# DIAGNijmegen/prostateMR_3D-CAD-csPCa

Measured on AMD Instinct MI355X. Metric: train-step volumes/sec (whole job), M1 (20,160,160,3), higher is better.
Workload: dtype bf16; 1 GPU; C3 M1 full hierarchical-probabilistic dense_skip+deep_supervision latents (3,2,1,0) (20,160,160,3); batch_per_gpu=2, global_batch=2, params=67254246, parallelism=dp1, hip_graph=True

## Files before the change

### prostatemr_3d-cad-cspca_amd/csrc/conv_mfma.h

```cpp
#pragma once
#include "common.h"
#include "gather.h"
#include "cdna4.h"

#define MF_MAX_TAPS 27
#define MF_MAX_CLASSES 8

struct MfmaP {
    const void* src[M1_MAX_SRC];
    int srcC[M1_MAX_SRC];
    int srcSeg[M1_MAX_SRC];
    int nsrc, CC, spt;
    int ID, IH, IW;
    void* out;
    int OC, OCn;
    int nout;
    void* outs[M1_MAX_SRC]; int outC[M1_MAX_SRC]; int outOff[M1_MAX_SRC + 1]; int outAcc[M1_MAX_SRC];
    int OD, OH, OW, N;
    const void* wp;
    const float* bias;
    const float* bias2; int bias_split;
    int mode, sd, sh, sw, pd, ph, pw;
    int nclasses;
    int cls_ntaps[MF_MAX_CLASSES], cls_first[MF_MAX_CLASSES], cls_kpad[MF_MAX_CLASSES];
    long long cls_woff[MF_MAX_CLASSES];
    signed char tdd[MF_MAX_TAPS], tdh[MF_MAX_TAPS], tdw[MF_MAX_TAPS];
    int tap_pk[MF_MAX_TAPS];
    int accumulate;
    int ksplit;
    float* acc32;
    long long slab_elems;
    int aligned;
    int korder;
    const void* ib_x;
    const float* ib_stats; const float* ib_gamma; const float* ib_beta; float ib_slope;
    int tps;
    float* stat_partial;
    int stat_tiles;
};

struct OutRef { void* base; int C, col, acc; };
__device__ __forceinline__ OutRef m1_out_ref(const MfmaP& p, int oc) {
    if (p.nout == 0) return OutRef{p.out, p.OC, oc, p.accumulate};
    int m = 0;
    while (m + 1 < p.nout && oc >= p.outOff[m + 1]) ++m;
    return OutRef{p.outs[m], p.outC[m], oc - p.outOff[m], p.outAcc[m]};
}

__device__ __forceinline__ float m1_bias_at(const MfmaP& p, int oc) {
    if (p.bias_split > 0 && oc >= p.bias_split) return p.bias2 ? p.bias2[oc - p.bias_split] : 0.f;
    return p.bias ? p.bias[oc] : 0.f;
}

template <typename T> struct MT;
template <> struct MT<bf16_t> { static constexpr int SEG = 8; };
template <> struct MT<float> { static constexpr int SEG = 4; };


bool m1_halo_conv_supported(const MfmaP& mp, int OCpad);
int m1_halo_conv_stat_parts(const MfmaP& mp, int OCpad);
int m1_halo_conv(const MfmaP& mp, int OCpad, hipStream_t st);

bool m1_pw_conv_supported(const MfmaP& mp, int OCpad, int BN);
int m1_pw_conv_stat_parts(const MfmaP& mp, int OCpad, int BN);
int m1_pw_conv(const MfmaP& mp, int OCpad, int BN, hipStream_t st);
```

### prostatemr_3d-cad-cspca_amd/csrc/conv_mfma.hip

```cpp
#include "common.h"
#include "gather.h"
#include "reduce.h"

#include "conv_mfma.h"
#include "conv_t3.h"
#include <stdlib.h>

template <typename T>
__device__ __forceinline__ uint4 load_partial_seg(const T* p, int n) {
    constexpr int SEG = MT<T>::SEG;
    union { uint4 v; T e[SEG]; } u;
    u.v = make_uint4(0, 0, 0, 0);
#pragma unroll
    for (int k = 0; k < SEG; ++k) if (k < n) u.e[k] = p[k];
    return u.v;
}

__device__ __forceinline__ unsigned lds_addr_of(const void* p) { return (unsigned)(unsigned long long)(lptr_t)p; }

template <typename T, int BM, int BN, int WM, int WN, int KC, bool GLDS, int KG = 1>
__global__ void __launch_bounds__(WM * WN * 64 * KG) conv_mfma_kernel(MfmaP p) {
#if defined(__HIP_DEVICE_COMPILE__)
    constexpr int NTHR = WM * WN * 64, NW = WM * WN;
    static_assert(KG == 1 || GLDS, "K groups: LDS-DMA path only");
    constexpr int SEG = MT<T>::SEG;
    constexpr int TM = BM / WM / 16, TN = BN / WN / 16;
    constexpr int A_BYTES = BM * 64, B_BYTES = BN * 64;
    constexpr int A_LD = BM * 4 / NTHR;
    constexpr int B_LD = (BN * 4 + NTHR - 1) / NTHR;
    static_assert((NW == 4 || NW == 8 || NW == 16) && (BM * 4) % NTHR == 0 && BN % 16 == 0, "tile config");

    extern __shared__ __attribute__((aligned(16))) unsigned char smem[];
    int4* rowinfo = reinterpret_cast<int4*>(smem);
    int* outrow = reinterpret_cast<int*>(rowinfo + BM);
    const T** s_src = reinterpret_cast<const T**>(outrow + BM);
    int* s_srcC = reinterpret_cast<int*>(s_src + M1_MAX_SRC);
    int* s_srcSeg = s_srcC + M1_MAX_SRC;
    int* s_tap = s_srcSeg + M1_MAX_SRC;
    int* s_tdl = s_tap + MF_MAX_TAPS;
    constexpr int TBL_BYTES = (BM * 20 + M1_MAX_SRC * 16 + 2 * MF_MAX_TAPS * 4 + 15) / 16 * 16;
    const int kg = KG > 1 ? __builtin_amdgcn_readfirstlane((int)threadIdx.x / NTHR) : 0;
    const int tid = KG > 1 ? (int)threadIdx.x - kg * NTHR : (int)threadIdx.x, lane = tid & 63, wave = tid >> 6;
    constexpr int GROUP_BYTES = 2 * KC * (A_BYTES + B_BYTES);
    unsigned char* A_s = smem + TBL_BYTES + kg * GROUP_BYTES;
    unsigned char* B_s = A_s + 2 * KC * A_BYTES;

    const int wm = wave / WN, wn = wave % WN;
    const int cls = blockIdx.y / p.ksplit, ksp = (blockIdx.y % p.ksplit) * KG + kg;
    const int oc0 = blockIdx.z * BN;

    int pdc = 0, phc = 0, pwc = 0, QD = p.OD, QH = p.OH, QW = p.OW;
    if (p.mode == 1) {
        pwc = cls % p.sw; phc = (cls / p.sw) % p.sh; pdc = cls / (p.sw * p.sh);
        QD = p.OD > pdc ? (p.OD - pdc + p.sd - 1) / p.sd : 0;
        QH = p.OH > phc ? (p.OH - phc + p.sh - 1) / p.sh : 0;
        QW = p.OW > pwc ? (p.OW - pwc + p.sw - 1) / p.sw : 0;
    }
    const long long QV = (long long)QD * QH * QW, Mtot = QV * p.N;
    const long long tile = (long long)(blockIdx.x & 7) * (gridDim.x >> 3) + (blockIdx.x >> 3);
    long long m0 = tile * BM, m_end = Mtot;
    if (p.tps > 0) {
        if (tile >= (long long)p.tps * p.N) return;
        const long long tn = tile / p.tps;
        m0 = tn * QV + (tile - tn * p.tps) * BM; m_end = (tn + 1) * QV;
    }
    if (m0 >= Mtot) return;

    for (int r = tid; r < BM; r += NTHR) {
        const long long m = m0 + r;
        int4 ri = make_int4(-1, 0, 0, 0); int orow = -1;
        if (m < m_end) {
            int n, qw, qh, qd;
            if (Mtot < (1ll << 31)) {
                const unsigned mm = (unsigned)m, qv = (unsigned)QV;
                n = (int)(mm / qv); const unsigned lin = mm - (unsigned)n * qv;
                const unsigned t1 = lin / (unsigned)QW; qw = (int)(lin - t1 * (unsigned)QW);
                qd = (int)(t1 / (unsigned)QH); qh = (int)(t1 - (unsigned)qd * (unsigned)QH);
            } else {
                n = (int)(m / QV); long long lin = m % QV;
                qw = (int)(lin % QW); lin /= QW; qh = (int)(lin % QH); qd = (int)(lin / QH);
            }
            if (p.mode == 0) {
                ri = make_int4(n, qd * p.sd - p.pd, qh * p.sh - p.ph, qw * p.sw - p.pw);
                orow = (int)m;
            } else {
                ri = make_int4(n, qd, qh, qw);
                orow = (int)((((long long)n * p.OD + qd * p.sd + pdc) * p.OH + qh * p.sh + phc) * p.OW + qw * p.sw + pwc);
            }
        }
        rowinfo[r] = ri; outrow[r] = orow;
    }
    if (tid < M1_MAX_SRC) { s_src[tid] = (const T*)p.src[tid]; s_srcC[tid] = p.srcC[tid]; s_srcSeg[tid] = p.srcSeg[tid]; }
    const int ntaps = p.cls_ntaps[cls], tfirst = p.cls_first[cls];
    if (tid < ntaps) {
        const int t = tfirst + tid;
        s_tap[tid] = ((int)p.tdd[t] & 0xff) | (((int)p.tdh[t] & 0xff) << 8) | (((int)p.tdw[t] & 0xff) << 16);
        s_tdl[tid] = ((int)p.tdd[t] * p.IH + (int)p.tdh[t]) * p.IW + (int)p.tdw[t];
    }
    __syncthreads();

    const int spt = p.spt;
    const int nseg = ntaps * spt;
    const int nchunks_all = (nseg + 3) >> 2;
    const int cps = (nchunks_all + p.ksplit * KG - 1) / (p.ksplit * KG);
    const int c_beg = ksp * cps;
    const int nchunks = (c_beg + cps <= nchunks_all ? cps : nchunks_all - c_beg);
    const int kpad = p.cls_kpad[cls];
    const T* wp = (const T*)p.wp + p.cls_woff[cls];

    f32x4_t acc[TM][TN];
#pragma unroll
    for (int i = 0; i < TM; ++i)
#pragma unroll
        for (int j = 0; j < TN; ++j) acc[i][j] = (f32x4_t){0.f, 0.f, 0.f, 0.f};

    uint4 ra[GLDS ? 1 : KC][GLDS ? 1 : A_LD], rb[GLDS ? 1 : KC][GLDS ? 1 : B_LD];
    const int lrow = tid >> 2;
    const int lseg = GLDS ? ((tid & 3) ^ ((-(tid >> 4)) & 3)) : (tid & 3);
    const int wave_u = __builtin_amdgcn_readfirstlane(wave);

    int st_tap = 0, st_s = 0, st_c = 0;
    const T* st_ptr[A_LD];
    auto st_set_tap = [&]() {
        const int tp = s_tap[st_tap];
        const int dd = (signed char)(tp & 0xff), dh = (signed char)((tp >> 8) & 0xff), dw = (signed char)((tp >> 16) & 0xff);
#pragma unroll
        for (int i = 0; i < A_LD; ++i) {
            const int4 ri = rowinfo[lrow + (NTHR / 4) * i];
            const int id = ri.y + dd, ih = ri.z + dh, iw = ri.w + dw;
            st_ptr[i] = nullptr;
            if (ri.x >= 0 && id >= 0 && id < p.ID && ih >= 0 && ih < p.IH && iw >= 0 && iw < p.IW) {
                const long long vox = (((long long)ri.x * p.ID + id) * p.IH + ih) * p.IW + iw;
                st_ptr[i] = s_src[st_s] + vox * s_srcC[st_s] + lseg * SEG;
            }
        }
    };
    constexpr unsigned OOB = 0x80000000u;
    unsigned b_vo[B_LD];
    unsigned rmask[A_LD]; int rvox[A_LD], rbyte[A_LD];
    int tap_db = 0;
    __amdgpu_buffer_rsrc_t rs_a = __builtin_amdgcn_make_buffer_rsrc((void*)p.src[0], 0, 0, 0x00020000);
    auto glds_set_member = [&]() {
        const int sC = __builtin_amdgcn_readfirstlane(s_srcC[st_s]);
#pragma unroll
        for (int i = 0; i < A_LD; ++i) rbyte[i] = (rvox[i] * sC + lseg * SEG) * (int)sizeof(T);
        rs_a = __builtin_amdgcn_make_buffer_rsrc((void*)p.src[__builtin_amdgcn_readfirstlane(st_s)], 0, 0x7fffffff, 0x00020000);
    };
    auto glds_set_tap = [&]() {
        tap_db = __builtin_amdgcn_readfirstlane(s_tdl[st_tap]) * __builtin_amdgcn_readfirstlane(s_srcC[st_s]) * (int)sizeof(T);
    };
    if constexpr (GLDS) {
        int4 ris[A_LD];
#pragma unroll
        for (int i = 0; i < A_LD; ++i) { ris[i] = rowinfo[lrow + (NTHR / 4) * i]; rmask[i] = 0; }
#pragma unroll 9
        for (int t = 0; t < ntaps; ++t) {
            const int tp = s_tap[t];
            const int dd = (signed char)(tp & 0xff), dh = (signed char)((tp >> 8) & 0xff), dw = (signed char)((tp >> 16) & 0xff);
#pragma unroll
            for (int i = 0; i < A_LD; ++i) {
                const bool ok = ris[i].x >= 0 && (unsigned)(ris[i].y + dd) < (unsigned)p.ID && (unsigned)(ris[i].z + dh) < (unsigned)p.IH &&
                                (unsigned)(ris[i].w + dw) < (unsigned)p.IW;
                rmask[i] |= (ok ? 1u : 0u) << t;
            }
        }
#pragma unroll
        for (int i = 0; i < A_LD; ++i) rvox[i] = ((ris[i].x * p.ID + ris[i].y) * p.IH + ris[i].z) * p.IW + ris[i].w;
    }
    if constexpr (GLDS) {
#pragma unroll
        for (int i = 0; i < B_LD; ++i) {
            const int e = tid + NTHR * i;
            b_vo[i] = (unsigned)(((oc0 + (e >> 2)) * kpad + lseg * SEG) * (int)sizeof(T));
        }
    }
    if (p.aligned && nchunks > 0) {
        const int cpt = spt >> 2;
        int c;
        if (p.korder == 2) { const int cg = c_beg / (2 * ntaps), rem = c_beg - cg * 2 * ntaps; st_tap = rem >> 1; c = (cg * 2 + (rem & 1)) * 4 * SEG; }
        else if (p.korder) { const int cg = c_beg / ntaps; st_tap = c_beg - cg * ntaps; c = cg * 4 * SEG; }
        else { st_tap = c_beg / cpt; c = (c_beg - st_tap * cpt) * 4 * SEG; }
        while (c >= s_srcC[st_s]) { c -= s_srcC[st_s]; ++st_s; }
        st_c = c;
        if constexpr (GLDS) { glds_set_member(); glds_set_tap(); } else st_set_tap();
    }

    auto prefetch_stage = [&](int sg) {
#pragma unroll
        for (int kc = 0; kc < KC; ++kc) {
            const int rel = sg * KC + kc;
            const int chunk = c_beg + rel;
            const bool live = rel < nchunks;
#pragma unroll
            for (int i = 0; i < B_LD; ++i) {
                const int e = tid + NTHR * i;
                uint4 v = make_uint4(0, 0, 0, 0);
                if (live && e < BN * 4)
                    v = *reinterpret_cast<const uint4*>(wp + (long long)(oc0 + (e >> 2)) * kpad + (long long)(chunk * 4 + (e & 3)) * SEG);
                rb[kc][i] = v;
            }
            if (!live) {
#pragma unroll
                for (int i = 0; i < A_LD; ++i) ra[kc][i] = make_uint4(0, 0, 0, 0);
            } else if (p.aligned) {
#pragma unroll
                for (int i = 0; i < A_LD; ++i)
                    ra[kc][i] = st_ptr[i] ? *reinterpret_cast<const uint4*>(st_ptr[i] + st_c) : make_uint4(0, 0, 0, 0);
                st_c += 4 * SEG;
                if (st_c >= s_srcC[st_s]) {
                    st_c = 0;
                    if (++st_s == p.nsrc) { st_s = 0; ++st_tap; }
                    if (st_tap < ntaps) st_set_tap();
                }
            } else {
                const int kseg = chunk * 4 + lseg;
                const T* sp = nullptr; int sC = 0, coff = 0, dd = 0, dh = 0, dw = 0;
                const bool kvalid = kseg < nseg;
                if (kvalid) {
                    const int tap_i = kseg / spt;
                    int cs = kseg - tap_i * spt, s = 0;
                    while (cs >= s_srcSeg[s]) { cs -= s_srcSeg[s]; ++s; }
                    sp = s_src[s]; sC = s_srcC[s]; coff = cs * SEG;
                    const int tp = s_tap[tap_i];
                    dd = (signed char)(tp & 0xff); dh = (signed char)((tp >> 8) & 0xff); dw = (signed char)((tp >> 16) & 0xff);
                }
#pragma unroll
                for (int i = 0; i < A_LD; ++i) {
                    const int4 ri = rowinfo[lrow + (NTHR / 4) * i];
                    uint4 v = make_uint4(0, 0, 0, 0);
                    const int id = ri.y + dd, ih = ri.z + dh, iw = ri.w + dw;
                    if (kvalid && coff < sC && ri.x >= 0 && id >= 0 && id < p.ID && ih >= 0 && ih < p.IH && iw >= 0 && iw < p.IW) {
                        const long long vox = (((long long)ri.x * p.ID + id) * p.IH + ih) * p.IW + iw;
                        if (sC % SEG == 0) v = *reinterpret_cast<const uint4*>(sp + vox * sC + coff);
                        else v = load_partial_seg<T>(sp + vox * sC + coff, sC - coff < SEG ? sC - coff : SEG);
                    }
                    ra[kc][i] = v;
                }
            }
        }
    };
    const __amdgpu_buffer_rsrc_t rs_b = __builtin_amdgcn_make_buffer_rsrc((void*)wp, 0, 0x7fffffff, 0x00020000);
    const __amdgpu_buffer_rsrc_t rs_0 = __builtin_amdgcn_make_buffer_rsrc((void*)wp, 0, 0, 0x00020000);
    auto issue_chunk = [&](int kc, int buf, int chunk, const __amdgpu_buffer_rsrc_t ra, const __amdgpu_buffer_rsrc_t rb) {
#pragma unroll
        for (int i = 0; i < B_LD; ++i)
            if ((NW * (i + 1)) * 64 <= BN * 4 || (wave_u + NW * i) * 64 < BN * 4)
                __builtin_amdgcn_raw_ptr_buffer_load_lds(rb, (lptr_t)(B_s + (buf * KC + kc) * B_BYTES + (wave_u + NW * i) * 1024), 16,
                                                         b_vo[i], chunk * 64, 0, 0);
#pragma unroll
        for (int i = 0; i < A_LD; ++i) {
            const unsigned vo = ((rmask[i] >> st_tap) & 1u) ? (unsigned)(rbyte[i] + tap_db) : OOB;
            __builtin_amdgcn_raw_ptr_buffer_load_lds(ra, (lptr_t)(A_s + (buf * KC + kc) * A_BYTES + (wave_u + NW * i) * 1024), 16,
                                                     vo, st_c * (int)sizeof(T), 0, 0);
        }
    };
    auto advance_chunk = [&]() {
        if (p.korder == 2) {
            if (((st_c / (4 * SEG)) & 1) == 0) st_c += 4 * SEG;
            else {
                st_c -= 4 * SEG;
                if (++st_tap == ntaps) {
                    st_tap = 0; st_c += 8 * SEG;
                    if (st_c >= s_srcC[st_s]) { st_c = 0; if (++st_s < p.nsrc) glds_set_member(); }
                }
                if (st_s < p.nsrc) glds_set_tap();
            }
        } else if (p.korder) {
            if (++st_tap == ntaps) {
                st_tap = 0; st_c += 4 * SEG;
                if (st_c >= s_srcC[st_s]) { st_c = 0; if (++st_s < p.nsrc) glds_set_member(); }
            }
            if (st_s < p.nsrc) glds_set_tap();
        } else {
            st_c += 4 * SEG;
            if (st_c >= s_srcC[st_s]) {
                st_c = 0;
                if (++st_s == p.nsrc) { st_s = 0; ++st_tap; }
                if (st_tap < ntaps) { glds_set_member(); glds_set_tap(); }
            }
        }
    };
    auto issue = [&](int sg, int buf) {
        const int rel0 = sg * KC;
        if (rel0 + KC <= nchunks) {
#pragma unroll
            for (int kc = 0; kc < KC; ++kc) { issue_chunk(kc, buf, c_beg + rel0 + kc, rs_a, rs_b); advance_chunk(); }
        } else {
#pragma unroll
            for (int kc = 0; kc < KC; ++kc) {
                const bool live = rel0 + kc < nchunks;
                issue_chunk(kc, buf, c_beg + rel0 + kc, live ? rs_a : rs_0, live ? rs_b : rs_0);
                if (live) advance_chunk();
            }
        }
    };
    auto stage = [&](int buf) {
#pragma unroll
        for (int kc = 0; kc < KC; ++kc) {
#pragma unroll
            for (int i = 0; i < A_LD; ++i) {
                const int row = lrow + (NTHR / 4) * i;
                *reinterpret_cast<uint4*>(A_s + (buf * KC + kc) * A_BYTES + row * 64 + m1_swz64(row, lseg) * 16) = ra[kc][i];
            }
#pragma unroll
            for (int i = 0; i < B_LD; ++i) {
                const int e = tid + NTHR * i;
                if (e < BN * 4) {
                    const int row = e >> 2;
                    *reinterpret_cast<uint4*>(B_s + (buf * KC + kc) * B_BYTES + row * 64 + m1_swz64(row, e & 3) * 16) = rb[kc][i];
                }
            }
        }
    };

    const int fr = lane & 15, fs = lane >> 4;
    const unsigned a_rd = lds_addr_of(A_s) + (wm * (BM / WM) + fr) * 64 + m1_swz64(fr, fs) * 16;
    const unsigned b_rd = lds_addr_of(B_s) + (wn * (BN / WN) + fr) * 64 + m1_swz64(fr, fs) * 16;
    const int nstages = KG > 1 ? (cps + KC - 1) / KC : (nchunks + KC - 1) / KC;
    if (nstages > 0) {
        if constexpr (GLDS) issue(0, 0);
        else { prefetch_stage(0); stage(0); }
    }
    __syncthreads();
    for (int it = 0; it < nstages; ++it) {
        const int buf = it & 1;
        if (it + 1 < nstages) { if constexpr (GLDS) issue(it + 1, buf ^ 1); else prefetch_stage(it + 1); }
        if constexpr (GLDS) {
            u32x4_t af[KC][TM], bfr[KC][TN];
            auto rd = [&](int kc) {
#pragma unroll
                for (int i = 0; i < TM; ++i) af[kc][i] = m1_lds_read128(a_rd + (buf * KC + kc) * A_BYTES + i * 1024);
#pragma unroll
                for (int j = 0; j < TN; ++j) bfr[kc][j] = m1_lds_read128(b_rd + (buf * KC + kc) * B_BYTES + j * 1024);
            };
            rd(0);
#pragma unroll
            for (int kc = 0; kc < KC; ++kc) {
                m1_lds_wait(af[kc][0]);
#pragma unroll
                for (int i = 1; i < TM; ++i) m1_lds_tie(af[kc][i]);
#pragma unroll
                for (int j = 0; j < TN; ++j) m1_lds_tie(bfr[kc][j]);
                if (kc + 1 < KC) rd(kc + 1);
                __builtin_amdgcn_sched_barrier(0);
#pragma unroll
                for (int i = 0; i < TM; ++i)
#pragma unroll
                    for (int j = 0; j < TN; ++j) {
                        if constexpr (sizeof(T) == 2) {
                            acc[i][j] = __builtin_amdgcn_mfma_f32_16x16x32_bf16(__builtin_bit_cast(bf16x8_t, af[kc][i]),
                                                                                __builtin_bit_cast(bf16x8_t, bfr[kc][j]), acc[i][j], 0, 0, 0);
                        } else {
#pragma unroll
                            for (int q = 0; q < 4; ++q)
                                acc[i][j] = __builtin_amdgcn_mfma_f32_16x16x4f32(__uint_as_float(af[kc][i][q]), __uint_as_float(bfr[kc][j][q]), acc[i][j], 0, 0, 0);
                        }
                    }
                if (kc + 1 < KC) __builtin_amdgcn_sched_barrier(0);
            }
        } else {
// ... 85 lines not shown
        constexpr int EPI_BYTES = (int)((BM * CP * sizeof(T) + 15) / 16 * 16), PIPE_BYTES = 2 * KC * (A_BYTES + B_BYTES) * KG;
        float* red = reinterpret_cast<float*>(A_s + (PIPE_BYTES > EPI_BYTES ? PIPE_BYTES : EPI_BYTES));
        constexpr int G = NTHR / BN;
        const int col = tid % BN, rg = tid / BN;
        float s = 0.f, ss = 0.f;
        if (p.ib_x) {
            const int oc = oc0 + col < p.OCn ? oc0 + col : 0, n = (int)(m0 / QV);
            const float mean = p.ib_stats[((long long)n * p.OC + oc) * 2], rstd = p.ib_stats[((long long)n * p.OC + oc) * 2 + 1];
            const float gm = p.ib_gamma[oc], bt = p.ib_beta[oc];
            const T* xb = (const T*)p.ib_x + oc;
            constexpr int RPT = (BM + G - 1) / G;
            if constexpr (RPT > 32) {
                for (int row = rg; row < BM; row += G) {
                    const int orow = outrow[row];
                    if (orow >= 0) {
                        const float xh = (Act<T>::ld(xb + (long long)orow * p.OC) - mean) * rstd;
                        const float dy = Act<T>::ld(C_s + row * CP + col) * lrelu_g(gm * xh + bt, p.ib_slope);
                        s += dy; ss += dy * xh;
                    }
                }
            } else {
            float xv[RPT];
#pragma unroll
            for (int i = 0; i < RPT; ++i) {
                const int row = rg + i * G;
                const int orow = row < BM ? outrow[row] : -1;
                xv[i] = orow >= 0 ? Act<T>::ld(xb + (long long)orow * p.OC) : 0.f;
            }
#pragma unroll
            for (int i = 0; i < RPT; ++i) {
                const int row = rg + i * G;
                if (row < BM && outrow[row] >= 0) {
                    const float xh = (xv[i] - mean) * rstd;
                    const float dy = Act<T>::ld(C_s + row * CP + col) * lrelu_g(gm * xh + bt, p.ib_slope);
                    s += dy; ss += dy * xh;
                }
            }
            }
        } else
        for (int row = rg; row < BM; row += G) {
            if (outrow[row] >= 0) { const float v = Act<T>::ld(C_s + row * CP + col); s += v; ss += v * v; }
        }
        red[tid * 2] = s; red[tid * 2 + 1] = ss;
        __syncthreads();
        if (rg == 0 && oc0 + col < p.OCn) {
            for (int q = 1; q < G; ++q) { s += red[(q * BN + col) * 2]; ss += red[(q * BN + col) * 2 + 1]; }
            float* dst = p.stat_partial + ((tile * p.OC) + oc0 + col) * 2;
            dst[0] = s; dst[1] = ss;
        }
    }
    constexpr int SPR = BN / SEG;
    for (int e = tid; e < BM * SPR; e += NTHR) {
        const int row = e / SPR, cs = e % SPR;
        const int orow = outrow[row];
        const int oc = oc0 + cs * SEG;
        if (orow < 0 || oc >= p.OCn) continue;
        const OutRef o = m1_out_ref(p, oc);
        if (!o.base) continue;
        uint4 v = *reinterpret_cast<const uint4*>(C_s + row * CP + cs * SEG);
        T* dst = (T*)o.base + (long long)orow * o.C + o.col;
        if (o.C % SEG != 0 || (p.nout == 0 && oc + SEG > p.OCn)) {
            union { uint4 q; T e[SEG]; } ve; ve.q = v;
#pragma unroll
            for (int k = 0; k < SEG; ++k) {
                if (oc + k < p.OCn) {
                    float a = Act<T>::ld(&ve.e[k]);
                    if (o.acc) a += Act<T>::ld(dst + k);
                    Act<T>::st(dst + k, a);
                }
            }
            continue;
        }
        if (o.acc) {
            float a[SEG], b[SEG];
            VecIO<T, SEG>::ld(reinterpret_cast<const T*>(&v), a);
            VecIO<T, SEG>::ld(dst, b);
#pragma unroll
            for (int k = 0; k < SEG; ++k) a[k] += b[k];
            VecIO<T, SEG>::st(dst, a);
        } else {
            *reinterpret_cast<uint4*>(dst) = v;
        }
    }
#endif
}

template <typename T, int BM, int BN, int KC, int NTHR, int KG = 1>
static constexpr size_t mfma_smem_bytes() {
    size_t tbl = (BM * 20 + M1_MAX_SRC * 16 + 2 * MF_MAX_TAPS * 4 + 15) / 16 * 16;
    size_t pipe = (size_t)KC * (2 * BM * 64 + 2 * BN * 64) * KG;
    size_t epi = ((size_t)BM * (BN + MT<T>::SEG) * sizeof(T) + 15) / 16 * 16;
    return tbl + (pipe > epi ? pipe : epi) + NTHR * 2 * sizeof(float);
}

struct PackP {
    const float* w; long long wST, wSC, wSO; int oc_off, cc_off, OCn, OCpad, CC;
    const float* w2; long long w2ST, w2SC, w2SO; int oc_split, c_split;
    int nsrc, spt, SEG; int srcC[M1_MAX_SRC], srcSeg[M1_MAX_SRC];
    int nclasses; int cls_ntaps[MF_MAX_CLASSES], cls_first[MF_MAX_CLASSES], cls_kpad[MF_MAX_CLASSES];
    long long cls_woff[MF_MAX_CLASSES];
    unsigned char wtap[MF_MAX_TAPS];
    int korder;
};
__device__ __forceinline__ bool pack_seg_pos(const PackP& p, int cls, int kseg, int* nvalid, int* wtap, int* chan) {
    int tap_i, seg;
    if (p.korder == 2) {
        const int chunk = kseg >> 2, nt = p.cls_ntaps[cls], cg = chunk / (2 * nt), rem = chunk - cg * 2 * nt;
        tap_i = rem >> 1; seg = (cg * 2 + (rem & 1)) * 4 + (kseg & 3);
    } else if (p.korder) {
        const int chunk = kseg >> 2, nt = p.cls_ntaps[cls], cg = chunk / nt;
        tap_i = chunk - cg * nt; seg = cg * 4 + (kseg & 3);
    } else { tap_i = kseg / p.spt; seg = kseg - tap_i * p.spt; }
    int c = 0, s = 0;
    while (s < p.nsrc && seg >= p.srcSeg[s]) { seg -= p.srcSeg[s]; c += p.srcC[s]; ++s; }
    if (s >= p.nsrc || tap_i >= p.cls_ntaps[cls]) { *nvalid = 0; return false; }
    const int rem = p.srcC[s] - seg * p.SEG;
    *nvalid = rem < p.SEG ? rem : p.SEG;
    *chan = c + seg * p.SEG;
    *wtap = p.wtap[p.cls_first[cls] + tap_i];
    return true;
}
#define M1_PACK_JOB_BYTES 512
#define M1_PACK_MAGIC 0x4d315031u
struct PackJob { PackP p; void* out; int dtype; unsigned magic; };
static_assert(sizeof(PackJob) <= M1_PACK_JOB_BYTES, "pack job record");

template <typename T>
__device__ __forceinline__ void pack_class_elems(const PackP& p, int cls, T* __restrict__ out, long long first, long long stride) {
    constexpr int SEG = MT<T>::SEG;
    const int kpad = p.cls_kpad[cls], nks = kpad / SEG;
    const bool oc_fast = p.wSO == 1;
    const int ocg = p.OCpad >> 4, ksg = (nks + 3) >> 2;
    const long long tot = oc_fast ? (long long)ocg * ksg * 64 : (long long)p.OCpad * nks;
    for (long long u = first; u < tot; u += stride) {
        int oc, kseg;
        if (oc_fast) {
            const long long grp = u >> 6; const int l = (int)(u & 63);
            oc = (int)(grp % ocg) * 16 + (l & 15); kseg = (int)(grp / ocg) * 4 + (l >> 4);
            if (kseg >= nks) continue;
        } else { oc = (int)(u / nks); kseg = (int)(u % nks); }
        int nvalid, wtap = 0, c = 0;
        pack_seg_pos(p, cls, kseg, &nvalid, &wtap, &c);
        if (oc >= p.OCn) nvalid = 0;
        const float* w = p.w; long long wST = p.wST, wSC = p.wSC, wSO = p.wSO; int ocl = oc + p.oc_off, cl = c + p.cc_off;
        if (p.w2 && ((p.oc_split > 0 && oc >= p.oc_split) || (p.c_split > 0 && c >= p.c_split))) {
            w = p.w2; wST = p.w2ST; wSC = p.w2SC; wSO = p.w2SO;
            if (p.oc_split > 0) ocl = oc - p.oc_split + p.oc_off; else cl = c - p.c_split;
        }
        const long long so = (long long)wtap * wST + (long long)cl * wSC + (long long)ocl * wSO;
        float v[SEG];
#pragma unroll
        for (int j = 0; j < SEG; ++j) v[j] = j < nvalid ? w[so + (long long)j * wSC] : 0.f;
        VecIO<T, SEG>::st(out + p.cls_woff[cls] + (long long)oc * kpad + (long long)kseg * SEG, v);
    }
}
template <typename T>
__global__ void pack_weights_kernel(PackP p, T* __restrict__ out, PackJob* __restrict__ job) {
    if (job && blockIdx.x == 0 && blockIdx.y == 0 && threadIdx.x == 0) {
        job->p = p; job->out = out; job->dtype = sizeof(T) == 2 ? M1_BF16 : M1_F32; job->magic = M1_PACK_MAGIC;
    }
    pack_class_elems<T>(p, blockIdx.y, out, (long long)blockIdx.x * blockDim.x + threadIdx.x, (long long)gridDim.x * blockDim.x);
}
__global__ void __launch_bounds__(256) pack_batch_kernel(const PackJob* const* __restrict__ jobs) {
    __shared__ PackJob j;
    const unsigned* src = reinterpret_cast<const unsigned*>(jobs[blockIdx.y]);
    for (int i = threadIdx.x; i < (int)(sizeof(PackJob) / 4); i += blockDim.x) reinterpret_cast<unsigned*>(&j)[i] = src[i];
// ... 146 lines not shown
        if (pl.ksplit < 1) pl.ksplit = 1;
        if (pl.ksplit > 32) pl.ksplit = 32;
    }
    return pl;
}
static inline long long spec_maxM(const GatherSpec& g) {
    if (g.mode == 0) return (long long)g.N * g.OD * g.OH * g.OW;
    return (long long)g.N * ((g.OD + g.sd - 1) / g.sd) * ((g.OH + g.sh - 1) / g.sh) * ((g.OW + g.sw - 1) / g.sw);
}
static inline int spec_ncls(const GatherSpec& g) { return g.mode == 1 ? g.sd * g.sh * g.sw : 1; }

bool m1_mfma_supported(const GatherSpec& g) {
    if (g.kd * g.kh * g.kw > MF_MAX_TAPS) return false;
    if (g.mode == 1 && g.sd * g.sh * g.sw > MF_MAX_CLASSES) return false;
    return true;
}

static inline int spec_spt(const GatherSpec& g, int SEG) {
    int s = 0; for (int i = 0; i < g.nsrc; ++i) s += (g.srcC[i] + SEG - 1) / SEG; return s;
}
static void build_classes(const GatherSpec& g, int CC, int SEG, int OCpad, MfmaP* mp, PackP* pp, long long* total_elems) {
    const int ncls = g.mode == 1 ? g.sd * g.sh * g.sw : 1;
    int t = 0; long long woff = 0;
    for (int c = 0; c < ncls; ++c) {
        const int pwc = g.mode == 1 ? c % g.sw : 0, phc = g.mode == 1 ? (c / g.sw) % g.sh : 0, pdc = g.mode == 1 ? c / (g.sw * g.sh) : 0;
        const int first = t;
        for (int a = 0; a < g.kd; ++a) {
            int od;
            if (g.mode == 0) od = a - 0; else { int v = pdc + g.pd - a; if (v % g.sd) continue; od = v / g.sd; }
            for (int b = 0; b < g.kh; ++b) {
                int oh;
                if (g.mode == 0) oh = b; else { int v = phc + g.ph - b; if (v % g.sh) continue; oh = v / g.sh; }
                for (int e = 0; e < g.kw; ++e) {
                    int ow;
                    if (g.mode == 0) ow = e; else { int v = pwc + g.pw - e; if (v % g.sw) continue; ow = v / g.sw; }
                    if (mp) { mp->tdd[t] = (signed char)od; mp->tdh[t] = (signed char)oh; mp->tdw[t] = (signed char)ow; }
                    if (pp) pp->wtap[t] = (unsigned char)((a * g.kh + b) * g.kw + e);
                    ++t;
                }
            }
        }
        const int nt = t - first;
        const int nseg = nt * spec_spt(g, SEG);
        const int kpad = ((nseg + 3) / 4) * 4 * SEG;
        if (mp) { mp->cls_ntaps[c] = nt; mp->cls_first[c] = first; mp->cls_kpad[c] = kpad; mp->cls_woff[c] = woff; }
        if (pp) { pp->cls_ntaps[c] = nt; pp->cls_first[c] = first; pp->cls_kpad[c] = kpad; pp->cls_woff[c] = woff; }
        woff += (long long)OCpad * kpad;
    }
    if (mp) mp->nclasses = ncls;
    if (pp) pp->nclasses = ncls;
    *total_elems = woff;
}

static inline int min_class_chunks(const GatherSpec& g, int CC, int SEG) {
    MfmaP tmp{}; long long tot = 0;
    build_classes(g, CC, SEG, 16, &tmp, nullptr, &tot);
    int mn = 1 << 30;
    for (int c = 0; c < tmp.nclasses; ++c) { int n = tmp.cls_kpad[c] / (4 * SEG); if (n < mn) mn = n; }
    return mn;
}
static inline size_t out_elems(const GatherSpec& g) { return (size_t)g.N * g.OD * g.OH * g.OW * g.OC; }

size_t m1_mfma_ws_bytes(const GatherSpec& g) {
    const int SEG = seg_of(g.dtype);
    int CC = 0; for (int i = 0; i < g.nsrc; ++i) CC += g.srcC[i];
    size_t best = 0;
    const bool maybe160 = g.dtype == M1_BF16 && g.mode == 0 && g.OC % 160 == 0 && g.OC <= 320;
    int t3bn = 0, t3ks = 1;
    const bool t3 = m1_ct3_plan(g, &t3bn, &t3ks);
    for (int v = 0; v < 3; ++v) {
        if ((v == 1 && !maybe160) || (v == 2 && !t3)) continue;
        Plan pl = make_plan(g.OC, spec_maxM(g), spec_ncls(g), min_class_chunks(g, CC, SEG), v == 1);
        if (v == 2) { pl.BN = t3bn; pl.BM = 256; pl.ksplit = t3ks; }
        const int BN = pl.BN, OCpad = (g.OC + BN - 1) / BN * BN;
        long long tot = 0;
        build_classes(g, CC, SEG, OCpad, nullptr, nullptr, &tot);
        size_t bytes = ((size_t)tot * (g.dtype == M1_BF16 ? 2 : 4) + 255) / 256 * 256;
        if (pl.ksplit > 1) bytes += out_elems(g) * sizeof(float) * pl.ksplit;
        if (bytes > best) best = bytes;
    }
    return best + 256 + M1_PACK_JOB_BYTES;
}

template <typename T, int BM, int BN, int WM, int WN, int KC>
static int launch_cfg_kc(const MfmaP& mp, long long maxM, int OCpad, hipStream_t st) {
    dim3 grid((unsigned)(cdiv_ll(cdiv_ll(maxM, BM), 8) * 8), mp.nclasses * mp.ksplit, OCpad / BN);
    const size_t smem = mfma_smem_bytes<T, BM, BN, KC, WM * WN * 64>();
    auto kern = mp.aligned ? conv_mfma_kernel<T, BM, BN, WM, WN, KC, true> : conv_mfma_kernel<T, BM, BN, WM, WN, KC, false>;
    if (smem > 48 * 1024 && m1_allow_dynamic_lds((const void*)kern, (int)smem) != M1_OK) return M1_ERR_LAUNCH;
    m1_note_kernel("conv_mfma:%dx%d:w%d:ks%d", BM, BN, WM * WN, mp.ksplit);
    hipLaunchKernelGGL(kern, grid, dim3(WM * WN * 64), smem, st, mp);
    return m1_check_launch();
}

template <typename T, int BM, int BN, int WM, int WN, int KG>
static int launch_cfg_kg(const MfmaP& mp, long long maxM, int OCpad, hipStream_t st) {
    constexpr size_t smem = mfma_smem_bytes<T, BM, BN, 2, WM * WN * 64, KG>();
    if constexpr (sizeof(T) != 2 || smem > 160 * 1024 - 256 || WM * WN * 64 * KG > 1024) return M1_ERR_UNSUPPORTED;
    else {
        dim3 grid((unsigned)(cdiv_ll(cdiv_ll(maxM, BM), 8) * 8), mp.nclasses * mp.ksplit, OCpad / BN);
        if (m1_allow_dynamic_lds((const void*)conv_mfma_kernel<T, BM, BN, WM, WN, 2, true, KG>, (int)smem) != M1_OK) return M1_ERR_LAUNCH;
        m1_note_kernel("conv_mfma:%dx%d:w%d:ks%d:kg%d", BM, BN, WM * WN, mp.ksplit, KG);
        hipLaunchKernelGGL((conv_mfma_kernel<T, BM, BN, WM, WN, 2, true, KG>), grid, dim3(WM * WN * 64 * KG), smem, st, mp);
        return m1_check_launch();
    }
}
static inline int mfma_kg_max(int BM, int BN, int nthr) {
    const int group = 2 * 2 * (BM + BN) * 64;
    int k = (150 * 1024) / group; if (k > 1024 / nthr) k = 1024 / nthr; if (k > 4) k = 4;
    return k >= 2 ? k : 0;
}

template <typename T, int BM, int BN, int WM, int WN>
static int launch_cfg(const MfmaP& mp, long long maxM, int OCpad, hipStream_t st, int kg = 1) {
    if (kg == 2) return launch_cfg_kg<T, BM, BN, WM, WN, 2>(mp, maxM, OCpad, st);
    if (kg == 3) return launch_cfg_kg<T, BM, BN, WM, WN, 3>(mp, maxM, OCpad, st);
    if (kg == 4) return launch_cfg_kg<T, BM, BN, WM, WN, 4>(mp, maxM, OCpad, st);
    int minchunks = 1 << 30;
    for (int c = 0; c < mp.nclasses; ++c) { const int n = mp.cls_kpad[c] / (4 * MT<T>::SEG) / mp.ksplit; if (n < minchunks) minchunks = n; }
    return minchunks >= 6 ? launch_cfg_kc<T, BM, BN, WM, WN, 2>(mp, maxM, OCpad, st)
                          : launch_cfg_kc<T, BM, BN, WM, WN, 1>(mp, maxM, OCpad, st);
}

template <typename T>
static int run_mfma(const GatherSpec& g, void* ws, int ws_packed, hipStream_t st) {
    constexpr int SEG = MT<T>::SEG;
    MfmaP mp{}; PackP pp{};
    int CC = 0;
    for (int i = 0; i < M1_MAX_SRC; ++i) {
        mp.src[i] = i < g.nsrc ? g.src[i] : nullptr; mp.srcC[i] = i < g.nsrc ? g.srcC[i] : (1 << 30);
        mp.srcSeg[i] = i < g.nsrc ? (g.srcC[i] + SEG - 1) / SEG : (1 << 30);
        pp.srcC[i] = i < g.nsrc ? g.srcC[i] : 0; pp.srcSeg[i] = i < g.nsrc ? (g.srcC[i] + SEG - 1) / SEG : 0;
        if (i < g.nsrc) CC += g.srcC[i];
    }
    mp.nsrc = g.nsrc; mp.CC = CC; mp.spt = spec_spt(g, SEG);
    pp.nsrc = g.nsrc; pp.spt = mp.spt; pp.SEG = SEG; mp.ID = g.ID; mp.IH = g.IH; mp.IW = g.IW; mp.out = g.out; mp.OC = g.OC; mp.OCn = g.OC;
    void* panel = reinterpret_cast<unsigned char*>(ws) + M1_PACK_JOB_BYTES;
    mp.OD = g.OD; mp.OH = g.OH; mp.OW = g.OW; mp.N = g.N; mp.wp = panel; mp.bias = g.bias; mp.mode = g.mode;
    mp.sd = g.sd; mp.sh = g.sh; mp.sw = g.sw; mp.pd = g.pd; mp.ph = g.ph; mp.pw = g.pw; mp.accumulate = g.accumulate;
    mp.bias2 = g.bias2; mp.bias_split = g.oc_split;
    mp.nout = g.nout; mp.outOff[0] = 0;
    for (int i = 0; i < g.nout; ++i) { mp.outs[i] = g.outs[i]; mp.outC[i] = g.outC[i]; mp.outAcc[i] = g.outAcc[i]; mp.outOff[i + 1] = mp.outOff[i] + g.outC[i]; }
    Plan pl = make_plan(g.OC, spec_maxM(g), spec_ncls(g), min_class_chunks(g, CC, SEG), want_bn160(g));
    int t3bn = 0, t3ks = 1;
    const bool t3 = sizeof(T) == 2 && m1_ct3_plan(g, &t3bn, &t3ks);
    if (t3) { pl.BN = t3bn; pl.BM = 256; pl.ksplit = t3ks; }
    int kgroups = 1;
    if (sizeof(T) == 2 && !t3 && pl.BM == 64 && (pl.BN == 64 || pl.BN == 128) && pl.ksplit >= 2 && M1_CFG("M1_MFMA_KG", 1)) {
        bool al = true;
        for (int i = 0; i < g.nsrc; ++i) al = al && g.srcC[i] % (4 * SEG) == 0;
        const int kmax = mfma_kg_max(64, pl.BN, 256);
        const long long tiles64 = cdiv_ll(spec_maxM(g), 64) * spec_ncls(g) * ((g.OC + pl.BN - 1) / pl.BN);
        if (al && kmax >= 2 && pl.ksplit <= 4 && tiles64 >= 200) { kgroups = pl.ksplit < kmax ? pl.ksplit : kmax; pl.ksplit = 1; }
    }
    const int BN = pl.BN, OCpad = (g.OC + BN - 1) / BN * BN;
    long long tot = 0;
    build_classes(g, CC, SEG, OCpad, &mp, &pp, &tot);
    mp.ksplit = pl.ksplit; mp.acc32 = nullptr; mp.aligned = 1; mp.stat_partial = nullptr; mp.stat_tiles = 0;
    const long long Vout = (long long)g.OD * g.OH * g.OW;
    int c8 = M1_CFG("M1_CONV8", 1);
    const bool use8 = !t3 && kgroups == 1 && c8 && BN == 128 && (pl.ksplit == 1 || (c8 >= 2 && pl.BM == 128)) &&
                      cdiv_ll(spec_maxM(g), 128) * spec_ncls(g) * (OCpad / 128) * pl.ksplit >= 160;
    const int bm_eff = t3 ? 256 : (use8 ? 128 : pl.BM);
    const int tiles_ps = t3 ? m1_ct3_tiles_per_sample(g.OD, g.OH, g.OW) : (int)cdiv_ll(Vout, bm_eff);
    const bool per_sample = !t3 && g.N > 1 && Vout % bm_eff != 0 && spec_ncls(g) == 1 && pl.ksplit == 1 && M1_CFG("M1_MFMA_TPS", 1) &&
                            (long long)tiles_ps * bm_eff * g.N < (1ll << 31);
    bool fuse_stats = g.stats_out && g.stats_ws && g.mode == 0 && pl.ksplit == 1 && (g.N == 1 || Vout % bm_eff == 0 || t3 || per_sample) &&
                      !g.accumulate;
    if (fuse_stats) { mp.stat_partial = g.stats_ws; mp.stat_tiles = tiles_ps; }
    const bool ib_want = g.ib_x && g.ib_partial && g.ib_nparts && !g.stats_out && !g.accumulate && g.nout <= 1 && spec_ncls(g) == 1 &&
                         (g.nout == 0 || (g.outs[0] && !g.outAcc[0] && g.outC[0] == g.OC));
    if (g.ib_nparts) *g.ib_nparts = 0;
    bool ib_epi = ib_want && pl.ksplit == 1 && (g.N == 1 || Vout % bm_eff == 0 || t3 || per_sample) && tiles_ps <= g.ib_cap;
    mp.tps = (per_sample && (fuse_stats || ib_epi)) ? tiles_ps : 0;
    if (ib_epi) {
        mp.stat_partial = g.ib_partial; mp.stat_tiles = tiles_ps;
        mp.ib_x = g.ib_x; mp.ib_stats = g.ib_stats; mp.ib_gamma = g.ib_gamma; mp.ib_beta = g.ib_beta; mp.ib_slope = g.ib_slope;
    }
    for (int i = 0; i < g.nsrc; ++i) if (g.srcC[i] % (4 * SEG)) mp.aligned = 0;
    for (int i = 0; i < g.nsrc; ++i)
        if ((long long)g.N * g.ID * g.IH * g.IW * g.srcC[i] * (long long)sizeof(T) >= (1ll << 31) - 4096) mp.aligned = 0;
    if (tot * (long long)sizeof(T) >= (1ll << 31) - 4096) mp.aligned = 0;
// ... 144 lines not shown
```

Before: 91.46 volumes/s.

## Schedule conv classes heavy-first and optionally pack classes into grouped blocks

Adds a host-side scheduler that reorders the sub-pixel phase classes of strided convolutions by chunk count, so the heaviest classes launch first. It also adds an optional kernel variant in which one block loops over several classes and reuses the row table when their dimensions match. The aim is to cut load-imbalance tail effects across the grid. By default only the heavy-first ordering is enabled; grouping is off unless M1_MFMA_CLS_GROUPS is set. The trade-off is extra template instantiations and a per-class loop with an added barrier in the grouped path.

```diff
diff --git a/prostatemr_3d-cad-cspca_amd/csrc/conv_mfma.h b/prostatemr_3d-cad-cspca_amd/csrc/conv_mfma.h
--- a/prostatemr_3d-cad-cspca_amd/csrc/conv_mfma.h
+++ b/prostatemr_3d-cad-cspca_amd/csrc/conv_mfma.h
@@ -1,10 +1,51 @@
 #pragma once
+
+#define MF_MAX_TAPS 27
+#define MF_MAX_CLASSES 8
+
+struct MfmaSched { int order[MF_MAX_CLASSES]; int ngroups; int first[MF_MAX_CLASSES + 1]; };
+#define MF_CLS_COST 16
+
+static inline void m1_mfma_class_schedule(int ncls, const int* chunks, int heavy_first, int ngroups, int cls_cost, MfmaSched* s) {
+    int idx[MF_MAX_CLASSES];
+    for (int i = 0; i < ncls; ++i) idx[i] = i;
+    for (int i = 1; i < ncls; ++i)
+        for (int j = i; j > 0 && chunks[idx[j]] > chunks[idx[j - 1]]; --j) { const int t = idx[j]; idx[j] = idx[j - 1]; idx[j - 1] = t; }
+    if (ngroups < 1 || ngroups >= ncls) {
+        s->ngroups = ncls;
+        for (int i = 0; i < ncls; ++i) { s->order[i] = heavy_first ? idx[i] : i; s->first[i] = i; }
+        s->first[ncls] = ncls;
+        return;
+    }
+    int load[MF_MAX_CLASSES] = {0}, cnt[MF_MAX_CLASSES] = {0}, mem[MF_MAX_CLASSES][MF_MAX_CLASSES];
+    for (int i = 0; i < ncls; ++i) {
+        int b = 0;
+        for (int q = 1; q < ngroups; ++q) if (load[q] < load[b]) b = q;
+        mem[b][cnt[b]++] = idx[i]; load[b] += chunks[idx[i]] + cls_cost;
+    }
+    int bins[MF_MAX_CLASSES];
+    for (int b = 0; b < ngroups; ++b) bins[b] = b;
+    if (heavy_first)
+        for (int i = 1; i < ngroups; ++i)
+            for (int j = i; j > 0 && load[bins[j]] > load[bins[j - 1]]; --j) { const int t = bins[j]; bins[j] = bins[j - 1]; bins[j - 1] = t; }
+    int n = 0;
+    for (int b = 0; b < ngroups; ++b) {
+        s->first[b] = n;
+        for (int q = 0; q < cnt[bins[b]]; ++q) s->order[n++] = mem[bins[b]][q];
+    }
+    s->first[ngroups] = n; s->ngroups = ngroups;
+}
+
+static inline int m1_mfma_class_groups(int ncls, long long tiles, long long slots) {
+    if (ncls < 2 || tiles < 1 || tiles * ncls < slots) return ncls;
+    const long long g = (slots + tiles - 1) / tiles;
+    return g < 1 ? 1 : (g > ncls ? ncls : (int)g);
+}
+
+#ifndef M1_MFMA_SCHED_ONLY
 #include "common.h"
 #include "gather.h"
 #include "cdna4.h"
-
-#define MF_MAX_TAPS 27
-#define MF_MAX_CLASSES 8
 
 struct MfmaP {
     const void* src[M1_MAX_SRC];
@@ -24,6 +65,8 @@
     int nclasses;
     int cls_ntaps[MF_MAX_CLASSES], cls_first[MF_MAX_CLASSES], cls_kpad[MF_MAX_CLASSES];
     long long cls_woff[MF_MAX_CLASSES];
+    int cls_order[MF_MAX_CLASSES];
+    int grp_first[MF_MAX_CLASSES + 1];
     signed char tdd[MF_MAX_TAPS], tdh[MF_MAX_TAPS], tdw[MF_MAX_TAPS];
     int tap_pk[MF_MAX_TAPS];
     int accumulate;
@@ -64,3 +107,4 @@
 bool m1_pw_conv_supported(const MfmaP& mp, int OCpad, int BN);
 int m1_pw_conv_stat_parts(const MfmaP& mp, int OCpad, int BN);
 int m1_pw_conv(const MfmaP& mp, int OCpad, int BN, hipStream_t st);
+#endif
diff --git a/prostatemr_3d-cad-cspca_amd/csrc/conv_mfma.hip b/prostatemr_3d-cad-cspca_amd/csrc/conv_mfma.hip
--- a/prostatemr_3d-cad-cspca_amd/csrc/conv_mfma.hip
+++ b/prostatemr_3d-cad-cspca_amd/csrc/conv_mfma.hip
@@ -18,11 +18,12 @@
 
 __device__ __forceinline__ unsigned lds_addr_of(const void* p) { return (unsigned)(unsigned long long)(lptr_t)p; }
 
-template <typename T, int BM, int BN, int WM, int WN, int KC, bool GLDS, int KG = 1>
-__global__ void __launch_bounds__(WM * WN * 64 * KG) conv_mfma_kernel(MfmaP p) {
+template <typename T, int BM, int BN, int WM, int WN, int KC, bool GLDS, int KG = 1, bool GRP = false>
+__global__ void __launch_bounds__(WM * WN * 64 * KG) conv_mfma_kernel(MfmaP p_arg) {
 #if defined(__HIP_DEVICE_COMPILE__)
     constexpr int NTHR = WM * WN * 64, NW = WM * WN;
     static_assert(KG == 1 || GLDS, "K groups: LDS-DMA path only");
+    static_assert(!GRP || KG == 1, "class groups: one K group");
     constexpr int SEG = MT<T>::SEG;
     constexpr int TM = BM / WM / 16, TN = BN / WN / 16;
     constexpr int A_BYTES = BM * 64, B_BYTES = BN * 64;
@@ -40,14 +41,24 @@
     int* s_tdl = s_tap + MF_MAX_TAPS;
     constexpr int TBL_BYTES = (BM * 20 + M1_MAX_SRC * 16 + 2 * MF_MAX_TAPS * 4 + 15) / 16 * 16;
     const int kg = KG > 1 ? __builtin_amdgcn_readfirstlane((int)threadIdx.x / NTHR) : 0;
-    const int tid = KG > 1 ? (int)threadIdx.x - kg * NTHR : (int)threadIdx.x, lane = tid & 63, wave = tid >> 6;
+    int tid_ = KG > 1 ? (int)threadIdx.x - kg * NTHR : (int)threadIdx.x;
     constexpr int GROUP_BYTES = 2 * KC * (A_BYTES + B_BYTES);
     unsigned char* A_s = smem + TBL_BYTES + kg * GROUP_BYTES;
     unsigned char* B_s = A_s + 2 * KC * A_BYTES;
 
+    const int ybin = blockIdx.y / p_arg.ksplit, ksp = (blockIdx.y % p_arg.ksplit) * KG + kg;
+    const int oc0 = blockIdx.z * BN;
+    int ci = GRP ? p_arg.grp_first[ybin] : ybin;
+    const int ci_end = GRP ? p_arg.grp_first[ybin + 1] : ybin + 1;
+    int dQD = -1, dQH = -1, dQW = -1;
+    do {
+    if constexpr (GRP) asm volatile("" : "+v"(tid_));
+    auto kp = __builtin_amdgcn_kernarg_segment_ptr();
+    if constexpr (GRP) asm volatile("" : "+s"(kp));
+    const MfmaP& p = GRP ? *(const MfmaP*)kp : p_arg;
+    const int tid = tid_, lane = tid & 63, wave = tid >> 6;
     const int wm = wave / WN, wn = wave % WN;
-    const int cls = blockIdx.y / p.ksplit, ksp = (blockIdx.y % p.ksplit) * KG + kg;
-    const int oc0 = blockIdx.z * BN;
+    const int cls = p.cls_order[ci];
 
     int pdc = 0, phc = 0, pwc = 0, QD = p.OD, QH = p.OH, QW = p.OW;
     if (p.mode == 1) {
@@ -64,8 +75,14 @@
         const long long tn = tile / p.tps;
         m0 = tn * QV + (tile - tn * p.tps) * BM; m_end = (tn + 1) * QV;
     }
-    if (m0 >= Mtot) return;
-
+    if (m0 >= Mtot) { if constexpr (GRP) continue; else return; }
+
+    if (GRP && QD == dQD && QH == dQH && QW == dQW) {
+        for (int r = tid; r < BM; r += NTHR) {
+            const int4 ri = rowinfo[r];
+            if (ri.x >= 0) outrow[r] = (int)((((long long)ri.x * p.OD + ri.y * p.sd + pdc) * p.OH + ri.z * p.sh + phc) * p.OW + ri.w * p.sw + pwc);
+        }
+    } else
     for (int r = tid; r < BM; r += NTHR) {
         const long long m = m0 + r;
         int4 ri = make_int4(-1, 0, 0, 0); int orow = -1;
@@ -90,6 +107,7 @@
         }
         rowinfo[r] = ri; outrow[r] = orow;
     }
+    dQD = QD; dQH = QH; dQW = QW;
     if (tid < M1_MAX_SRC) { s_src[tid] = (const T*)p.src[tid]; s_srcC[tid] = p.srcC[tid]; s_srcSeg[tid] = p.srcSeg[tid]; }
     const int ntaps = p.cls_ntaps[cls], tfirst = p.cls_first[cls];
     if (tid < ntaps) {
@@ -100,6 +118,7 @@
     __syncthreads();
 
     const int spt = p.spt;
+    const int nsrc = p.nsrc, korder = p.korder;
     const int nseg = ntaps * spt;
     const int nchunks_all = (nseg + 3) >> 2;
     const int cps = (nchunks_all + p.ksplit * KG - 1) / (p.ksplit * KG);
@@ -177,8 +196,8 @@
     if (p.aligned && nchunks > 0) {
         const int cpt = spt >> 2;
         int c;
-        if (p.korder == 2) { const int cg = c_beg / (2 * ntaps), rem = c_beg - cg * 2 * ntaps; st_tap = rem >> 1; c = (cg * 2 + (rem & 1)) * 4 * SEG; }
-        else if (p.korder) { const int cg = c_beg / ntaps; st_tap = c_beg - cg * ntaps; c = cg * 4 * SEG; }
+        if (korder == 2) { const int cg = c_beg / (2 * ntaps), rem = c_beg - cg * 2 * ntaps; st_tap = rem >> 1; c = (cg * 2 + (rem & 1)) * 4 * SEG; }
+        else if (korder) { const int cg = c_beg / ntaps; st_tap = c_beg - cg * ntaps; c = cg * 4 * SEG; }
         else { st_tap = c_beg / cpt; c = (c_beg - st_tap * cpt) * 4 * SEG; }
         while (c >= s_srcC[st_s]) { c -= s_srcC[st_s]; ++st_s; }
         st_c = c;
@@ -209,7 +228,7 @@
                 st_c += 4 * SEG;
                 if (st_c >= s_srcC[st_s]) {
                     st_c = 0;
-                    if (++st_s == p.nsrc) { st_s = 0; ++st_tap; }
+                    if (++st_s == nsrc) { st_s = 0; ++st_tap; }
                     if (st_tap < ntaps) st_set_tap();
                 }
             } else {
@@ -255,27 +274,27 @@
         }
     };
     auto advance_chunk = [&]() {
-        if (p.korder == 2) {
+        if (korder == 2) {
             if (((st_c / (4 * SEG)) & 1) == 0) st_c += 4 * SEG;
             else {
                 st_c -= 4 * SEG;
                 if (++st_tap == ntaps) {
                     st_tap = 0; st_c += 8 * SEG;
-                    if (st_c >= s_srcC[st_s]) { st_c = 0; if (++st_s < p.nsrc) glds_set_member(); }
+                    if (st_c >= s_srcC[st_s]) { st_c = 0; if (++st_s < nsrc) glds_set_member(); }
                 }
-                if (st_s < p.nsrc) glds_set_tap();
-            }
-        } else if (p.korder) {
+                if (st_s < nsrc) glds_set_tap();
+            }
+        } else if (korder) {
             if (++st_tap == ntaps) {
                 st_tap = 0; st_c += 4 * SEG;
-                if (st_c >= s_srcC[st_s]) { st_c = 0; if (++st_s < p.nsrc) glds_set_member(); }
-            }
-            if (st_s < p.nsrc) glds_set_tap();
+                if (st_c >= s_srcC[st_s]) { st_c = 0; if (++st_s < nsrc) glds_set_member(); }
+            }
+            if (st_s < nsrc) glds_set_tap();
         } else {
             st_c += 4 * SEG;
             if (st_c >= s_srcC[st_s]) {
                 st_c = 0;
-                if (++st_s == p.nsrc) { st_s = 0; ++st_tap; }
+                if (++st_s == nsrc) { st_s = 0; ++st_tap; }
                 if (st_tap < ntaps) { glds_set_member(); glds_set_tap(); }
             }
         }
@@ -527,6 +546,8 @@
             *reinterpret_cast<uint4*>(dst) = v;
         }
     }
+    if constexpr (GRP) __syncthreads();
+    } while (GRP && ++ci < ci_end);
 #endif
 }
 
@@ -839,22 +860,59 @@
     return best + 256 + M1_PACK_JOB_BYTES;
 }
 
+static int mfma_schedule(MfmaP& mp, int seg, long long tiles, long long slots) {
+    int chunks[MF_MAX_CLASSES];
+    for (int c = 0; c < mp.nclasses; ++c) chunks[c] = mp.cls_kpad[c] / (4 * seg);
+    const int heavy = M1_CFG("M1_MFMA_CLS_ORDER", 1) ? 1 : 0;
+    int G = mp.nclasses;
+    if (tiles > 0 && mp.mode == 1 && mp.nclasses > 1 && mp.ksplit == 1) {
+        const int gs = M1_CFG("M1_MFMA_CLS_GROUPS", 0);
+        if (gs == 1) G = m1_mfma_class_groups(mp.nclasses, tiles, slots);
+        else if (gs >= 2) G = gs < mp.nclasses ? gs : mp.nclasses;
+    }
+    MfmaSched s;
+    m1_mfma_class_schedule(mp.nclasses, chunks, heavy, G, MF_CLS_COST, &s);
+    for (int c = 0; c < mp.nclasses; ++c) mp.cls_order[c] = s.order[c];
+    for (int b = 0; b <= s.ngroups; ++b) mp.grp_first[b] = s.first[b];
+    { int lg = M1_CFG("M1_MFMA_LOG", 0);
+      if (lg && mp.nclasses > 1) {
+          fprintf(stderr, "mfma: classes %d tiles %lld slots %lld bins %d:", mp.nclasses, tiles, slots, s.ngroups);
+          for (int b = 0; b < s.ngroups; ++b) {
+              fprintf(stderr, " {");
+              for (int i = s.first[b]; i < s.first[b + 1]; ++i) fprintf(stderr, "%s%d/%dt", i > s.first[b] ? " " : "", s.order[i], mp.cls_ntaps[s.order[i]]);
+              fprintf(stderr, "}");
+          }
+          fprintf(stderr, "\n");
+      } }
+    return s.ngroups;
+}
+
 template <typename T, int BM, int BN, int WM, int WN, int KC>
-static int launch_cfg_kc(const MfmaP& mp, long long maxM, int OCpad, hipStream_t st) {
-    dim3 grid((unsigned)(cdiv_ll(cdiv_ll(maxM, BM), 8) * 8), mp.nclasses * mp.ksplit, OCpad / BN);
-    const size_t smem = mfma_smem_bytes<T, BM, BN, KC, WM * WN * 64>();
+static int launch_cfg_kc(const MfmaP& mp_in, long long maxM, int OCpad, hipStream_t st) {
+    constexpr int NTHR = WM * WN * 64;
+    const size_t smem = mfma_smem_bytes<T, BM, BN, KC, NTHR>();
+    constexpr bool kGroups = BN >= 32 && BN <= 128;
+    MfmaP mp = mp_in;
+    const long long xt = cdiv_ll(maxM, BM);
+    long long per_cu = (long long)(160 * 1024 / smem); if (per_cu > 2048 / NTHR) per_cu = 2048 / NTHR;
+    const int bins = mfma_schedule(mp, MT<T>::SEG, kGroups && mp.aligned ? xt * (OCpad / BN) : 0, 256 * per_cu);
+    const bool grouped = bins < mp.nclasses;
+    dim3 grid((unsigned)(cdiv_ll(xt, 8) * 8), bins * mp.ksplit, OCpad / BN);
     auto kern = mp.aligned ? conv_mfma_kernel<T, BM, BN, WM, WN, KC, true> : conv_mfma_kernel<T, BM, BN, WM, WN, KC, false>;
+    if constexpr (kGroups) { if (grouped) kern = conv_mfma_kernel<T, BM, BN, WM, WN, KC, true, 1, true>; }
     if (smem > 48 * 1024 && m1_allow_dynamic_lds((const void*)kern, (int)smem) != M1_OK) return M1_ERR_LAUNCH;
     m1_note_kernel("conv_mfma:%dx%d:w%d:ks%d", BM, BN, WM * WN, mp.ksplit);
-    hipLaunchKernelGGL(kern, grid, dim3(WM * WN * 64), smem, st, mp);
+    hipLaunchKernelGGL(kern, grid, dim3(NTHR), smem, st, mp);
     return m1_check_launch();
 }
 
 template <typename T, int BM, int BN, int WM, int WN, int KG>
-static int launch_cfg_kg(const MfmaP& mp, long long maxM, int OCpad, hipStream_t st) {
+static int launch_cfg_kg(const MfmaP& mp_in, long long maxM, int OCpad, hipStream_t st) {
     constexpr size_t smem = mfma_smem_bytes<T, BM, BN, 2, WM * WN * 64, KG>();
     if constexpr (sizeof(T) != 2 || smem > 160 * 1024 - 256 || WM * WN * 64 * KG > 1024) return M1_ERR_UNSUPPORTED;
     else {
+        MfmaP mp = mp_in;
+        mfma_schedule(mp, MT<T>::SEG, 0, 0);
         dim3 grid((unsigned)(cdiv_ll(cdiv_ll(maxM, BM), 8) * 8), mp.nclasses * mp.ksplit, OCpad / BN);
         if (m1_allow_dynamic_lds((const void*)conv_mfma_kernel<T, BM, BN, WM, WN, 2, true, KG>, (int)smem) != M1_OK) return M1_ERR_LAUNCH;
         m1_note_kernel("conv_mfma:%dx%d:w%d:ks%d:kg%d", BM, BN, WM * WN, mp.ksplit, KG);
```

Measured after the change: 91.36 volumes/s. No clear change (-0.1%).
